# caomw/BundleAdjustmentMatlab

Measured on AMD Instinct MI355X. Metric: LM iterations/sec + observations/sec, 1000-cam/500k-pt synthetic, higher is better.
Workload: dtype f64; 1 GPU; cfg3: 1000 cams x 500000 pts x 3000000 obs, fix_calibration (num_a=6), full LM pass per step, one linearisation per step; cameras=1000, points=500000, observations=3000000, parallelism=point-shard x1

## Files before the change

bundleadjustmentmatlab_amd/bundle.py:

```python
from __future__ import annotations

import ctypes
import numpy as np

from ._lib import (ALLREDUCE_FN, LOSSES, MODEL_EUCLIDEAN, MODEL_PROJECTIVE, NKERNELS, ON_PASS_FN,
                   VlgbaOptions,
                   VlgbaProblem, VlgbaResectProblem, VlgbaStats,
                   VlgbaStepInfo, c_dp, c_ip, c_up, check, lib)

__all__ = ["bundle_euclid", "bundle_euclid_nomex", "bundle_euclid_obs", "BundleAdjuster",
           "bundle_euclid_resect",
           "parse_options", "pivot_mask",
           "mex_bundle_1_XABeUVWeAeB", "mex_bundle_2_Se_", "mex_bundle_3_db_new"]


def _F(a):
    return np.asfortranarray(a, dtype=np.float64)


def _dp(a):
    return a.ctypes.data_as(c_dp)


def pivot_mask(pivot, m):
# ... 320 lines not shown
        check(self._L.vlgba_set_timing(self._h, int(on)), "vlgba_set_timing")

    def kernel_ms(self, reset=True):
        n = NKERNELS
        ms = np.zeros(n)
        calls = (ctypes.c_longlong * n)()
        check(self._L.vlgba_kernel_ms(self._h, _dp(ms), calls, int(reset)), "vlgba_kernel_ms")
        return {self._L.vlgba_kernel_name(k).decode(): (float(ms[k]), int(calls[k]))
                for k in range(n) if calls[k] > 0}

    PLAN_KEYS = ("obs", "points", "cameras", "num_a", "chunks", "chunk_slots",
                 "chunk_eslots", "groups", "group_slots", "group_eslots", "blocks",
                 "tiles", "cr_levels", "cr_elim", "cr_keep", "ordered", "schur_terms",
                 "blob_words", "mfma", "cr_rows", "mfma_groups", "reordered", "long_points",
                 "nd_arcs", "nd_sep_tiles", "solve_flops_factor", "solve_flops_syrk",
                 "solve_flops_back", "env_runner_runs")

    def plan_info(self):
        n = len(self.PLAN_KEYS)
        buf = (ctypes.c_longlong * n)()
        rc = self._L.vlgba_plan_info(self._h, buf, n)
        check(min(rc, 0), "vlgba_plan_info")
        return dict(zip(self.PLAN_KEYS, [int(v) for v in buf]))

    def phase_ms(self):
        ms = np.zeros(7)
        check(self._L.vlgba_phase_ms(self._h, _dp(ms)), "vlgba_phase_ms")
        return dict(zip(["linearize", "camera_reduce", "damp_y", "schur", "assemble",
                         "cholesky_solve", "update"], ms.tolist()))


# ... 181 lines not shown
```

bundleadjustmentmatlab_amd/csrc/ba_chol.hip:

```cpp
#include "ba_internal.h"

#include <algorithm>
#include <atomic>
#include <mutex>
#include <cstdio>
#include <utility>
#include <climits>
#include <cstdlib>
#include <vector>

#define NB 64
#define LP 66

typedef double d4 __attribute__((ext_vector_type(4)));

__device__ __forceinline__ void load_tile(const double *__restrict__ S, long long lds, int ti,
                                          int tj, double *T)
{
    const double *base = S + (long long)NB * ti + lds * (long long)NB * tj;
    const int r = threadIdx.x & 63, c0 = threadIdx.x >> 6;
    double v[16];
#pragma unroll
    for (int u = 0; u < 16; u++) v[u] = base[r + lds * (c0 + 4 * u)];
#pragma unroll
// ... 2149 lines not shown
        }
    }
    __syncthreads();
}

__device__ __forceinline__ void cr32_publish(unsigned *flag, unsigned epoch, int nflags = 1)
{
    asm volatile("s_waitcnt vmcnt(0)" ::: "memory");
    __syncthreads();
    if (threadIdx.x < nflags)
        __hip_atomic_store((gu32_t *)(flag + threadIdx.x), epoch, __ATOMIC_RELAXED,
                           __HIP_MEMORY_SCOPE_AGENT);
}


__global__ __launch_bounds__(256) void k_cr32_fused(double *S, long long lds, int TB, long long ld,
                                                    const int *__restrict__ elim,
                                                    const int *__restrict__ frec,
                                                    const int *__restrict__ srec, int nt,
                                                    double *linv, double *crL, double *rhs,
                                                    double *y, double *x, unsigned *flag,
                                                    unsigned long long *xg, unsigned epoch,
                                                    double *status, cr32_fplan P)
{
    CR32_LDS_DECL;
    CR_ST(0);
    const int b = blockIdx.x;
    int L = 0;
    while (L < P.nl && b >= P.b0[L + 1]) L++;
    auto fw = [&](int lev, int t, int r) { return 5 * (lev * nt + t) + r; };
    if (L == 0) {
        const int xr = P.l0two ? b / 2 : b / 3;
        const int role = P.l0two ? ((b & 1) ? 2 : 4) : b % 3;
        const int e = elim[3 * xr], p = elim[3 * xr + 1], q = elim[3 * xr + 2];
        CR_ST(1);
        if (!((role == 1 && p < 0) || (role == 2 && q < 0)))
            cr32_factor_body<true>(sh, S, lds, TB, ld, e, p, q, role, nt, linv, crL, rhs, y,
                                   status);
// ... 59 lines not shown
        if (!skip)
            cr32_level_body<true>(sh, S, lds, TB, ld, k, p, q, em, ep, role, nt, linv, crL, rhs,
                                  y, status, mid, BA_CR_PW ? &pw : nullptr);
        CR_ST(2);
        cr32_publish(flag + fw(L, k, role == 3 ? 4 : role), epoch);
        CR_ST(3);
        return;
    }
    const int rec = P.nrec - 1 - (b - P.b0[P.nl]);
    int Le = 0;
    while (Le + 1 < P.nl && rec >= P.eofs[Le + 1]) Le++;
    const int e = elim[3 * rec], p = elim[3 * rec + 1], q = elim[3 * rec + 2];
    const int w[8] = {fw(Le, e, 0), fw(Le, e, 1), fw(Le, e, 2), 0, 0, 0, 0, 0};
    cr32_wait_flags(flag, 3, w, epoch, status);
    CR_ST(1);
    cr32_back_body<true>(sh, e, p, q, nt, TB, ld, linv, crL, y, x, xg, epoch, status);
    CR_ST(2);
    CR_ST(3);
}

__global__ __launch_bounds__(256) void k_cr_back(const int *__restrict__ elim, int nt,
                                                 const double *__restrict__ linv,
                                                 const double *__restrict__ crL,
                                                 const double *__restrict__ y,
                                                 double *__restrict__ x)
{
    __shared__ double Ls[NB * LP];
    __shared__ double t[NB], u[NB];
    __shared__ double part[4][NB];
    const int tid = threadIdx.x;
    const int e = elim[3 * blockIdx.x], p = elim[3 * blockIdx.x + 1], q = elim[3 * blockIdx.x + 2];
    const long long T2 = (long long)NB * NB;
// ... 912 lines not shown
        KT_E(d, KT_BACKWARD);
        return -(int)hipGetLastError();
    }
    for (int k = nt - 1; k >= 0; k--) {
        const int j0 = d->h_tfirst[k];
        KT_B(d);
        k_backward<<<k - j0 + 1, 256, 0, d->stream>>>(d->S, L, k, j0, d->linv, d->ywork, x);
        KT_E(d, KT_BACKWARD);
    }
    return -(int)hipGetLastError();
}

int ba_chol_solve(ba_dev *d, int nospin)
{
    const int nt = d->nt;
    const size_t smem3 = sizeof(double) * 3 * NB * LP;
    TRY_RC(ba_ensure_dyn_lds((const void *)k_factor_step, smem3));
    TRY_RC(ba_ensure_dyn_lds((const void *)k_cr_factor, smem3));
    TRY_RC(ba_ensure_dyn_lds((const void *)k_cr_update, smem3));
    if (d->dense_solve == 3) {
        KT_B(d);
        k_chol_seq<<<1, 256, 0, d->stream>>>(d->S, d->lds, (int)d->ld, d->rhs, d->da,
                                             d->scal + 4);
        KT_E(d, KT_FACTOR);
        return -(int)hipGetLastError();
    }
    if (d->cr_nlev > 0 && d->cr32 && d->cr_fused && d->crflag && !nospin) {
        const int nl = d->cr_nlev, nrec = d->cr_eptr_h[nl];
        cr32_fplan P{};
        P.nl = nl;
        P.nrec = nrec;
        P.l0two = 3 * d->cr_eptr_h[1] > d->ncu;
        P.b0[0] = 0;
        P.b0[1] = (P.l0two ? 2 : 3) * d->cr_eptr_h[1];
        for (int l = 1; l < nl; l++) {
            const int nf = d->crf_ptr_h[l + 1] - d->crf_ptr_h[l];
            const int ns = d->crs_ptr_h[l + 1] - d->crs_ptr_h[l];
            P.fofs[l] = d->crf_ptr_h[l];
            P.sofs[l] = d->crs_ptr_h[l];
            P.b0[l + 1] = P.b0[l] + 3 * nf + ns;
        }
        P.sofs[nl] = d->crs_ptr_h[nl];
        for (int l = 0; l <= nl; l++) P.eofs[l] = d->cr_eptr_h[l];
        if (++d->back_epoch == 0) d->back_epoch = 1;
        KT_B(d);
        k_cr32_fused<<<P.b0[nl] + nrec, 256, 0, d->stream>>>(
            d->S, d->lds, d->tb32, d->ld, d->cr_elim, d->crf, d->crs, d->nt32, d->linv, d->crL,
            d->rhs, d->ywork, d->da, d->crflag, d->xgran, d->back_epoch, d->scal + 4, P);
        KT_E(d, KT_CR_FACTOR);
        return -(int)hipGetLastError();
    }
    if (d->cr_nlev > 0 && d->cr32) {
        const int ncu32 = d->ncu;
        const int n32 = d->nt32, TB = d->tb32;
        {
            const int ne = d->cr_eptr_h[1];
            const int fs = 3 * ne <= 2 * ncu32;
            KT_B(d);
            k_cr32_factor<<<fs ? 3 * ne : ne, 256, 0, d->stream>>>(
                d->S, d->lds, TB, d->ld, d->cr_elim, n32, d->linv, d->crL, d->rhs, d->ywork,
                d->scal + 4, fs);
            KT_E(d, KT_CR_FACTOR);
        }
// ... 148 lines not shown
```

bundleadjustmentmatlab_amd/csrc/ba_internal.h:

```cpp
#pragma once
#include <hip/hip_runtime.h>
#include <cstddef>
#include <cstdint>

#define VLGBA_CHECK(x)                                                              \
    do {                                                                            \
        hipError_t err__ = (x);                                                     \
        if (err__ != hipSuccess) return -(int)err__;                                \
    } while (0)

enum {
    KT_ROT, KT_LIN, KT_CAMRED, KT_DAMP, KT_SCHUR, KT_SCHUR_CHUNK, KT_SCHUR_RED,
    KT_ASSEMBLE, KT_FACTOR, KT_SYRK, KT_BACKWARD, KT_CAMUPD, KT_PTUPD, KT_CR_FACTOR,
    KT_CR_UPDATE, KT_CR_BACK, KT_SCHUR_MF, KT_LIN_UPD, KT_N
};
#define KT_MAX_EV 8192
struct ba_ktimer {
    int on;
    int nev;
    int ncreated;
    hipEvent_t ev[KT_MAX_EV];
    int kid[KT_MAX_EV / 2];
    double ms[KT_N];
    long long calls[KT_N];
// ... 71 lines not shown
    int *tb_ptr, *tb_blk;
    int n_env;
    int dense_solve;
    int cr_nlev;
    int *cr_eptr_h, *cr_kptr_h;
    int *cr_elim, *cr_keep;
    double *crL;
    int cr32, tb32, nt32;
    int *crf, *crs;
    int *crf_ptr_h, *crs_ptr_h;
    unsigned long long *xgran;
    unsigned back_epoch;
    unsigned *crflag;
    int cr_fused;
    int asm_direct_ok, asm_direct;
    int nd_np;
    int nd_grouped;
    int nd_a0[BA_ND_MAX + 1];
    long long slds;
    int *nd_crow;
    int *nd_prow;
    int *nd_rowsrc;
    double *nd_rhs, *nd_x;
    int nd_npair, nd_nrec;
    int *nd_pair;
    int *nd_pptr;
    int *nd_rec;
    int *nd_klist;
    double *nd_part;
    double fl_factor, fl_syrk, fl_back;
// ... 22 lines not shown
    double *chsse;
    int fused;
    double *W2, *V2, *eB2, *upart2, *chsse2;
    int ns, nes;
    int ch_max_terms, ch_max_slots;
    long long nterm_fast;
    long long blob_words;
    int ngrp, ngs, nge;
    int grp_max_s, grp_max_e;
    unsigned *blob;
    int *ch_blob, *ch_obase;
    int *ch_cam;
    unsigned char *obs_lpt;
    int max_blob;
    int ngrp_mf;
    int nch_reg, nl, p_long;
    int *seg_pt, *seg_long;
    int *long_pt, *long_o0, *long_seg0;
    int *long_ebase;
    int *cam_lptr, *cam_lobs, *cam_ltrk;
    int max_lcam;
    int long_o0_h;
    double *ylong;
    int *lpair_ptr;
    int2 *lpair;
    int *lblk;
    int nlb;
    double *vseg;
    double *dpg_long;
    int mf_max_s, mf_max_e, mf_max_blob;
// ... 100 lines not shown
```

bundleadjustmentmatlab_amd/csrc/ba_kernels.hip:

```cpp
#include "ba_internal.h"
#include "ba_camera.h"
#include "vlg_math.h"
#include "../../include/vlgba.h"

typedef double d4 __attribute__((ext_vector_type(4)));

#ifdef BA_STAMPS
__device__ unsigned long long g_stamp[32];
#define STAMP_DECL unsigned long long st_prev_ = __builtin_amdgcn_s_memtime()
#define STAMP(i)                                                                    \
    do {                                                                            \
        if (threadIdx.x == 0) {                                                     \
            const unsigned long long t_ = __builtin_amdgcn_s_memtime();             \
            atomicAdd(&g_stamp[i], t_ - st_prev_);                                  \
            st_prev_ = t_;                                                          \
        }                                                                           \
    } while (0)
extern "C" int vlgba_debug_stamps(unsigned long long *out, int reset)
{
    if (hipMemcpyFromSymbol(out, HIP_SYMBOL(g_stamp), sizeof(g_stamp)) != hipSuccess) return -1;
    if (reset) {
        unsigned long long z[32] = {};
        if (hipMemcpyToSymbol(HIP_SYMBOL(g_stamp), z, sizeof(z)) != hipSuccess) return -1;
    }
// ... 1087 lines not shown
template <int Q> __device__ __forceinline__ double row16_bcast_c(double v)
{
    const long long u = __builtin_bit_cast(long long, v);
    const long long r = __builtin_amdgcn_mov_dpp(u, 0x150 + Q, 0xf, 0xf, true);
    return __builtin_bit_cast(double, r);
}
#ifndef BA_MF_WAVES
#define BA_MF_WAVES 3
#endif
template <int NA>
__global__ __launch_bounds__(256, (NA == 6) ? BA_MF_WAVES : 1) void k_schur_mfma(
    const int *__restrict__ grp_ch, const int *__restrict__ grp_gs,
    const int *__restrict__ grp_ge, const int *__restrict__ ch_pt,
    const int *__restrict__ ch_obase, const int *__restrict__ ch_blob,
    const unsigned *__restrict__ blob, const double *__restrict__ W,
    const double *__restrict__ Vinv, const double *__restrict__ eB, int nobs_all, int n_all,
    int gcap, int ecap, double *__restrict__ spart, double *__restrict__ epart, int ngrp,
    ba_camred cred)
{
    if ((int)blockIdx.x >= ngrp) {
        camera_reduce_wg<NA>((int)blockIdx.x - ngrp, cred);
        return;
    }
    constexpr int WS = 3 * NA;
    constexpr int RT = BA_MF_RT(NA);
    constexpr int NTL = RT * (RT + 1) / 2;
    extern __shared__ __attribute__((aligned(16))) double sm[];
    double *gacc = sm;
    double *geacc = gacc + gcap * NA * NA;
    unsigned *rec = (unsigned *)(geacc + ecap * NA);
    __shared__ int gp0[BA_GROUP_CH + 1], gob[BA_GROUP_CH + 1], gbo[BA_GROUP_CH + 1];
    const int g = ngrp - 1 - (int)blockIdx.x;
    const int tid = threadIdx.x, lane = tid & 63, wv = tid >> 6;
    const int li = lane & 15, lk = lane >> 4;
    const int c0 = grp_ch[g], nc = grp_ch[g + 1] - c0;
    const int gs0 = grp_gs[g], ngs = grp_gs[g + 1] - gs0;
    const int ge0 = grp_ge[g], nge = grp_ge[g + 1] - ge0;
    const int rb0 = ch_blob[c0], nrw = ch_blob[c0 + nc] - rb0;
    for (int q = tid; q < ngs * NA * NA; q += 256) gacc[q] = 0.0;
    for (int q = tid; q < nge * NA; q += 256) geacc[q] = 0.0;
    for (int q = tid; q < nrw; q += 256) rec[q] = blob[rb0 + q];
    for (int q = tid; q <= nc; q += 256) {
        gp0[q] = ch_pt[c0 + q];
        gob[q] = ch_obase[c0 + q];
        gbo[q] = ch_blob[c0 + q] - rb0;
    }
    __syncthreads();
    int ccs[RT], crr[RT];
#pragma unroll
    for (int t = 0; t < RT; t++) {
        ccs[t] = (16 * t + li) / NA;
        crr[t] = (16 * t + li) % NA;
    }
// ... 870 lines not shown
            b_new[3 * (size_t)i + r] = b[3 * (size_t)i + r] + dbr;
            dpg += dbr * (lambda * dbr + eB[3 * (size_t)i + r]);
        }
        dpg_long[l] = dpg;
    }
}

struct ba_sum3 {
    const double *part[3];
    int n[3];
    double *out[3];
    const double *scal;
    double *hres;
    double seq;
    unsigned *cnt;
};

__global__ __launch_bounds__(1024) void k_sum_parts3(ba_sum3 a)
{
    const double *part = a.part[blockIdx.x];
    const int nparts = a.n[blockIdx.x];
    double v0 = 0.0, v1 = 0.0, v2 = 0.0, v3 = 0.0;
    int q = threadIdx.x;
    for (; q + 3 * 1024 < nparts; q += 4 * 1024) {
        v0 += part[q];
        v1 += part[q + 1024];
        v2 += part[q + 2 * 1024];
        v3 += part[q + 3 * 1024];
    }
    for (; q < nparts; q += 1024) v0 += part[q];
    block_sum_to<1024>((v0 + v1) + (v2 + v3), a.out[blockIdx.x]);
    if (a.hres && threadIdx.x == 0) {
        __threadfence();
        if (atomicAdd(a.cnt, 1u) == 2u) {
            __threadfence();
            const volatile double *sc = a.scal;
// ... 145 lines not shown
                           d->blk_jk, d->blk_ptr, d->term, d->Y, d->W, d->t, d->U, d->eA, d->nb,
                           lambda, d->schur_owner, d->sblk, d->rhs)));
    KT_E(d, KT_SCHUR);
    return -(int)hipGetLastError();
}

#ifndef BA_SCHUR_TWO_STREAMS
#define BA_SCHUR_TWO_STREAMS 1
#endif
template <int NA>
static int launch_schur_fast(ba_dev *d, double lambda)
{
    const bool two = BA_SCHUR_TWO_STREAMS && d->ngrp_mf > 0 && d->ngrp > d->ngrp_mf &&
                     !d->join_pending && d->side && !(d->kt && d->kt->on);
    if (d->ngrp_mf > 0) {
        KT_B(d);
        k_point_vinv<NA><<<(d->n + 255) / 256, 256, 0, d->stream>>>(d->V, d->n, lambda, d->Vinv);
        KT_E(d, KT_DAMP);
        if (two) VLGBA_CHECK(hipEventRecord(d->ev_fork, d->stream));
        const size_t sm2 = sizeof(double) * (d->mf_max_s * NA * NA + d->mf_max_e * NA) +
                           sizeof(unsigned) * (size_t)d->mf_max_blob;
        TRY_RC(ba_ensure_dyn_lds((const void *)k_schur_mfma<NA>, sm2));
        const int ncr = d->camred_pending ? d->m + 1 : 0;
        d->camred_pending = 0;
        KT_B(d);
        k_schur_mfma<NA><<<d->ngrp_mf + ncr, 256, sm2, d->stream>>>(
            d->grp_ch, d->grp_gs, d->grp_ge, d->ch_pt, d->ch_obase, d->ch_blob, d->blob, d->W,
            d->Vinv, d->eB, d->N, d->n, d->mf_max_s, d->mf_max_e, d->spart, d->epart,
            d->ngrp_mf, d->camred);
        KT_E(d, KT_SCHUR_MF);
    }
    if (d->ngrp > d->ngrp_mf) {
        const int gcap = d->grp_max_s, ecap = d->grp_max_e, bcap = d->max_blob;
        size_t smem = sizeof(double) * (2 * BA_CH_OBS * 3 * NA + BA_CH_PTS * 12 +
                                        gcap * NA * NA + ecap * NA) +
                      sizeof(unsigned) * bcap;
        smem = (smem + 15) & ~(size_t)15;
        TRY_RC(ba_ensure_dyn_lds((const void *)k_schur_group<NA>, smem));
        hipStream_t s0 = d->stream;
        if (two) {
            VLGBA_CHECK(hipStreamWaitEvent(d->side, d->ev_fork, 0));
            d->stream = d->side;
        }
        KT_B(d);
// ... 86 lines not shown
    const int g = grid_for(d->n, 256, 1 << 30);
    BA_DISPATCH(d->na, (k_point_yeb<NA><<<g, 256, 0, d->stream>>>(d->pt_ptr, d->Y, d->eB, d->n,
                                                                    d->t)));
    return -(int)hipGetLastError();
}

int ba_launch_assemble(ba_dev *d)
{
    if (d->asm_direct) return 0;
    KT_B(d);
    TRY_RC(ba_assemble_tiles(d));
    KT_E(d, KT_ASSEMBLE);
    return 0;
}

static int launch_update_fused(ba_dev *d, double lambda, ba_flags f)
{
    const int gc = (d->m + 63) / 64;
    KT_B(d);
    const double lam_dpg = d->dpg_lambda ? lambda : 0.0;
    BA_DISPATCH(d->na, (k_camera_update<NA><<<gc, 320, 0, d->stream>>>(
                           d->a, d->da, d->eA, d->m, lam_dpg, d->a_new, d->rot_new,
                           d->part)));
    KT_E(d, KT_CAMUPD);
    KT_B(d);
    if (d->nl > 0)
        BA_DISPATCH(d->na, (k_long_db<NA><<<d->nl, 256, 0, d->stream>>>(
                               d->long_pt, d->long_o0, d->obs_cam, d->W, d->da, d->eB,
                               d->Vinv, d->b, d->ndb, lambda, d->db, d->b_new,
                               d->dpg_long)));
    const ba_upd u{d->W, d->da, d->eB, d->Vinv, d->b, d->ndb, lambda, d->db, d->b_new,
                   d->chsse2 + 2 * (size_t)d->nch, d->seg_long, d->long_o0, d->dpg_long};
    BA_DISPATCH(d->na, (lin_chunk_launch<NA>(d, f, d->a_new, d->rot_new, d->b_new, d->W2,
                                             d->V2, d->eB2, d->upart2, d->chsse2, &u)));
    if (d->nl > 0)
        k_long_vsum<<<d->nl, 64, 0, d->stream>>>(d->long_pt, d->long_seg0, d->vseg, d->V2,
                                                 d->eB2);
    KT_E(d, KT_LIN_UPD);
    ba_sum3 s3 = {{d->chsse2, d->chsse2 + 2 * (size_t)d->nch, d->part},
                  {d->nch, d->nch, gc},
                  {d->scal + 1, d->scal + 3, d->scal + 2},
                  d->scal, nullptr, 0.0, d->pub_cnt};
    if (d->publish_req) {
        d->seq++;
        s3.hres = d->hres_dev;
        s3.seq = (double)d->seq;
        d->publish_req = 0;
        d->published = 1;
    }
    k_sum_parts3<<<3, 1024, 0, d->stream>>>(s3);
    return -(int)hipGetLastError();
}

int ba_launch_update(ba_dev *d, double lambda, ba_flags f)
{
    if (d->fused) return launch_update_fused(d, lambda, f);
    const int gc = (d->m + 63) / 64;
    KT_B(d);
    const double lam_dpg = d->dpg_lambda ? lambda : 0.0;
    BA_DISPATCH(d->na, (k_camera_update<NA><<<gc, 320, 0, d->stream>>>(
                           d->a, d->da, d->eA, d->m, lam_dpg, d->a_new, d->rot_new,
                           d->part)));
    KT_E(d, KT_CAMUPD);
    if (!d->ordered && d->nch > 0 && !d->obs_vis && !d->xh_out) {
        KT_B(d);
        if (d->nl > 0)
            BA_DISPATCH(d->na, (k_long_db<NA><<<d->nl, 256, 0, d->stream>>>(
                                   d->long_pt, d->long_o0, d->obs_cam, d->W, d->da, d->eB,
                                   d->Vinv, d->b, d->ndb, lambda, d->db, d->b_new,
                                   d->dpg_long)));
        if (d->loss_kind) {
            const ba_loss ls{d->loss_kind, d->loss_scale};
            BA_DISPATCH(d->na, (k_point_update_chunk_loss<NA><<<d->nch, 256, 0, d->stream>>>(
                                   d->ch_pt, d->ch_obase, d->pt_ptr, d->obs_cam, d->obs_lpt,
                                   d->obs_x, d->K4, d->W, d->da, d->eB, d->Vinv, d->b,
                                   d->a_new, d->rot_new, d->ndb, lambda, d->db, d->b_new,
                                   d->chsse + d->nch, d->chsse + 2 * (size_t)d->nch,
                                   d->nch_reg, d->seg_pt, d->seg_long, d->long_o0,
                                   d->dpg_long, ls)));
        } else {
            BA_DISPATCH(d->na, (k_point_update_chunk<NA><<<d->nch, 256, 0, d->stream>>>(
                                   d->ch_pt, d->ch_obase, d->pt_ptr, d->obs_cam, d->obs_lpt,
                                   d->obs_x, d->K4, d->W, d->da, d->eB, d->Vinv, d->b,
                                   d->a_new, d->rot_new, d->ndb, lambda, d->db, d->b_new,
                                   d->chsse + d->nch, d->chsse + 2 * (size_t)d->nch,
                                   d->nch_reg, d->seg_pt, d->seg_long, d->long_o0,
                                   d->dpg_long)));
        }
        KT_E(d, KT_PTUPD);
        ba_sum3 s3 = {{d->chsse + d->nch, d->chsse + 2 * (size_t)d->nch, d->part},
                      {d->nch, d->nch, gc},
                      {d->scal + 1, d->scal + 3, d->scal + 2},
                      d->scal, nullptr, 0.0, d->pub_cnt};
        if (d->publish_req) {
            d->seq++;
            s3.hres = d->hres_dev;
            s3.seq = (double)d->seq;
            d->publish_req = 0;
            d->published = 1;
        }
        k_sum_parts3<<<3, 1024, 0, d->stream>>>(s3);
        return -(int)hipGetLastError();
    }
    k_sum_parts<<<1, BA_SUM_BS, 0, d->stream>>>(d->part, gc, d->scal + 2);
    const int g = grid_for(d->n, 256, PT_GRID_CAP);
    KT_B(d);
    BA_DISPATCH(d->na, (k_point_update<NA><<<g, 256, 0, d->stream>>>(
                           d->pt_ptr, d->obs_cam, d->obs_x, d->K4, d->W, d->da, d->eB, d->Vinv,
// ... 86 lines not shown
```

bundleadjustmentmatlab_amd/csrc/ba_solver.cpp:

```cpp
#include "ba_internal.h"
#include "../../include/vlgba.h"

#include <rccl/rccl.h>
#include <climits>
#include <rocsolver/rocsolver.h>

#include <dlfcn.h>
#include <unistd.h>
#include <cstdlib>
#include <string>

#include <algorithm>
#include <atomic>
#include <chrono>
#include <cmath>
#include <condition_variable>
#include <functional>
#include <cstdio>
#include <cstring>
#include <mutex>
#include <unordered_map>
#include <map>
#include <new>
#include <numeric>
// ... 1492 lines not shown
            TRY(ctx_alloc(c, &d.vseg, 12 * (size_t)plan.nseg));
            TRY(ctx_alloc(c, &d.dpg_long, (size_t)d.nl));
        }
        d.ns = (int)plan.slot_blk.size();
        d.nes = (int)plan.eslot_optr.size() - 1;
        d.ch_max_terms = plan.max_terms;
        d.ch_max_slots = plan.max_slots;
        d.nterm_fast = plan.n_terms;
        d.blob_words = (long long)plan.blob.size();
        d.ngrp = (int)plan.grp_ch.size() - 1;
        d.ngrp_mf = plan.ngrp_mf;
        d.max_blob = plan.max_blob;
        d.mf_max_blob = plan.mf_max_blob;
        d.mf_max_s = plan.mf_max_s;
        d.mf_max_e = plan.mf_max_e;
        pb.add(&d.blob, plan.blob);
        pb.add(&d.ch_blob, plan.ch_blob);
        pb.add(&d.ch_obase, plan.ch_obase);
        std::vector<unsigned char> lpt(d.N > 0 ? d.N : 1, 0);
        for (size_t ch = 0; ch + 1 < plan.ch_pt.size(); ch++)
            for (int i = plan.ch_pt[ch]; i < plan.ch_pt[ch + 1]; i++)
                for (int o = lptr[i]; o < lptr[i + 1]; o++)
                    lpt[o] = (unsigned char)(i - plan.ch_pt[ch]);
        const size_t nchk = plan.ch_obase.size() - 1;
        std::vector<int> ccam(2 * std::max<size_t>(nchk, 1), 0);
        for (size_t ch = 0; ch < nchk; ch++) {
            int lo = INT_MAX, hi = -1;
            for (int o = plan.ch_obase[ch]; o < plan.ch_obase[ch + 1]; o++) {
                lo = std::min(lo, lcam[o]);
                hi = std::max(hi, lcam[o]);
// ... 61 lines not shown
        TRY(ctx_alloc(c, &lp_cnt, (size_t)d.nb + 1));
        TRY(ctx_alloc(c, &d.lpair_ptr, (size_t)d.nb + 1));
        TRY(ba_launch_long_pairs(&d, 0, lp_cnt));
    }
    TRY(ctx_alloc(c, &d.sblk, (size_t)na * na * d.nb + d.lds + 1));
    d.rhs = d.sblk + (size_t)na * na * d.nb;
    if (!stage_mode) {
        TRY(ctx_alloc(c, &d.da, (size_t)d.lds));
        ST_MARK("allocs");
        TRY(ba_chol_setup(&d, hb.jk.data(), d.nb));
        ST_MARK("chol_setup");
        const char *ad = std::getenv("VLGBA_ASM_DIRECT");
        d.asm_direct = d.asm_direct_ok && !(ad && ad[0] == '0') && fast && !d.ordered &&
                       c->world == 1 && !c->comm && d.nl == 0 && d.cr_nlev > 0 && d.cr32 &&
                       d.nd_np == 0;
    } else {
        TRY(ctx_alloc(c, &d.da, (size_t)d.lds));
    }
    TRY(ctx_alloc(c, &d.part, 3 * (size_t)BA_PART_MAX));
    TRY(ctx_alloc(c, &d.scal, 8));
    if (p->num_obs > 0 || true) {
        TRY(upload(d.obs_cam, lcam.data(), d.N, s));
        TRY(upload(d.pt_ptr, lptr.data(), d.n + 1, s));
        TRY(upload(d.cam_ptr, cptr.data(), p->m + 1, s));
        TRY(upload(d.cam_obs, cobs.data(), d.N, s));
        TRY(upload(d.obs_x, h.x.data() + 2 * o0, 2 * (size_t)d.N, s));
        if (p->K) TRY(upload(d.K4, p->K, 4 * (size_t)p->m, s));
        else VLGBA_CHECK(hipMemsetAsync(d.K4, 0, sizeof(double) * 4 * p->m, s));
        TRY(upload(d.blk_ptr, hb.ptr.data(), hb.ptr.size(), s));
        TRY(upload(d.term, hb.term.data(), hb.term.size(), s));
// ... 346 lines not shown
    int info = 0;
    {
        std::lock_guard<std::mutex> lk(g_rs_mu);
        if (rs->set_stream(hdl, d.stream) != rocblas_status_success ||
            rs->potrf(hdl, rocblas_fill_lower, (rocblas_int)ld, c->pinv_S, (rocblas_int)ld,
                      c->pinv_info) != rocblas_status_success)
            return VLGBA_E_ARG;
        VLGBA_CHECK(hipMemcpyAsync(&info, c->pinv_info, sizeof info, hipMemcpyDeviceToHost,
                                   d.stream));
        VLGBA_CHECK(hipStreamSynchronize(d.stream));
        if (info != 0) return 1;
        if (rs->potrs(hdl, rocblas_fill_lower, (rocblas_int)ld, 1, c->pinv_S, (rocblas_int)ld,
                      c->pinv_e, (rocblas_int)ld) != rocblas_status_success)
            return VLGBA_E_ARG;
    }
    VLGBA_CHECK(hipMemcpyAsync(d.da, c->pinv_e, sizeof(double) * ld, hipMemcpyDeviceToDevice,
                               d.stream));
    d.publish_req = 0;
    d.published = 0;
    TRY(ba_launch_update(&d, lam, c->flags));
    if (d.parity) TRY(ba_launch_parity_new_sums(&d, lam));
    TRY(collect_scalars(c, false, hs));
    c->nd_retries++;
    if (c->rank == 0 && !std::getenv("VLGBA_QUIET"))
        std::fprintf(stderr, "[vlgba] non-positive pivot in the nested-dissection order: the "
                             "natural-order Cholesky (dpotrf) took the pass\n");
    return 0;
}

static int pinv_fallback(vlgba_ctx *c, double lam, double hs[6])
// ... 10 lines not shown
    {
        std::lock_guard<std::mutex> lk(g_rs_mu);
        if (rs->set_stream(hdl, d.stream) != rocblas_status_success ||
            rs->syevd(hdl, rocblas_evect_original, rocblas_fill_lower, (rocblas_int)ld,
                      c->pinv_S, (rocblas_int)ld, c->pinv_ev, c->pinv_e,
                      c->pinv_info) != rocblas_status_success)
            return VLGBA_E_ARG;
        VLGBA_CHECK(hipStreamSynchronize(d.stream));
    }
    {
        int info = 0;
        VLGBA_CHECK(hipMemcpy(&info, c->pinv_info, sizeof info, hipMemcpyDeviceToHost));
        if (info != 0) return VLGBA_E_ARG;
    }
    TRY(ba_pinv_apply(&d, c->pinv_S, c->pinv_ev, ld, d.rhs, c->pinv_w, d.da));
    d.publish_req = 0;
    d.published = 0;
    TRY(ba_launch_update(&d, lam, c->flags));
    if (d.parity) TRY(ba_launch_parity_new_sums(&d, lam));
    TRY(collect_scalars(c, false, hs));
    c->pinv_used++;
    if (c->rank == 0 && !std::getenv("VLGBA_QUIET"))
        std::fprintf(stderr,
                     "[vlgba] non-positive pivot: da = pinv(S) e_ by dsyevd on the dense "
                     "%lld x %lld S (%.1f MB of device memory), %.3f s\n",
                     ld, ld, 8e-6 * (double)ld * (double)ld,
                     std::chrono::duration<double>(std::chrono::steady_clock::now() - t0).count());
    return 0;
}

// ... 732 lines not shown

int vlgba_plan_info(vlgba_ctx *c, long long *info, int len)
{
    if (!c || !info) return VLGBA_E_ARG;
    const ba_dev &d = c->d;
    const long long ne = d.cr_nlev ? d.cr_eptr_h[d.cr_nlev] : 0;
    const long long nk = d.cr_nlev ? d.cr_kptr_h[d.cr_nlev] : 0;
    const long long v[VLGBA_NPLAN] = {d.N,   d.n,    d.m,   d.na,         d.nch,  d.ns,
                                      d.nes, d.ngrp, d.ngs, d.nge,        d.nb,   d.nt,
                                      d.cr_nlev, ne, nk,    d.ordered,    d.ordered ? d.T : d.nterm_fast,
                                      d.blob_words, d.mfma,
                                      d.cr_nlev ? (d.cr32 ? d.tb32 : 64) : 0,
                                      d.ngrp_mf, c->pperm.empty() ? 0 : 1, d.nl, d.nd_np,
                                      d.nd_np ? d.nt - d.nd_a0[d.nd_np] : 0,
                                      (long long)d.fl_factor, (long long)d.fl_syrk,
                                      (long long)d.fl_back, d.runner_runs};
    for (int k = 0; k < len && k < VLGBA_NPLAN; k++) info[k] = v[k];
    return VLGBA_NPLAN;
}

int vlgba_phase_ms(vlgba_ctx *c, double *ms7)
{
    if (!c || !ms7) return VLGBA_E_ARG;
    for (int q = 0; q < 7; q++) ms7[q] = c->phase_ms[q];
    return 0;
}

int vlgba_sync(vlgba_ctx *c)
{
    if (!c) return VLGBA_E_ARG;
    TRY(ctx_enter(c));
// ... 247 lines not shown
        const size_t p = (size_t)pt[q] + (size_t)n * cam[q];
        ox[2 * q] = X[2 * p];
        ox[2 * q + 1] = X[2 * p + 1];
        std::memcpy(hW.data() + bs * q, W + bs * p, sizeof(double) * bs);
    }
    vlgba_problem pr = {m, n, num_a, N, pt.data(), cam.data(), ox.data(), K, 0.0, model};
    vlgba_ctx *c = nullptr;
    TRY(ctx_create(&pr, nullptr, &c, true, true, true));
    ba_dev &d = c->d;
    int rc = 0;
    do {
        if ((rc = ctx_alloc(c, &d.xh_out, 2 * (size_t)N))) break;
        if ((rc = ctx_alloc(c, &d.obs_vis, (size_t)N))) break;
        if ((rc = upload(d.obs_vis, ov.data(), ov.size(), d.stream))) break;
        if ((rc = upload(d.W, hW.data(), hW.size(), d.stream))) break;
        if ((rc = upload(d.da, da, (size_t)d.ld, d.stream))) break;
        if ((rc = upload(d.eB, eB, 3 * (size_t)n, d.stream))) break;
        if ((rc = upload(d.Vinv, Vinv, 9 * (size_t)n, d.stream))) break;
        if ((rc = upload(d.a, a, (size_t)d.ld, d.stream))) break;
        if ((rc = upload(d.b, b, 3 * (size_t)n, d.stream))) break;
        VLGBA_CHECK(hipMemsetAsync(d.eA, 0, sizeof(double) * d.ld, d.stream));
        if ((rc = ba_launch_update(&d, 0.0, ba_flags{}))) break;
        if ((rc = download(db, d.db, 3 * (size_t)n, d.stream))) break;
        if ((rc = download(a_new, d.a_new, (size_t)d.ld, d.stream))) break;
        if ((rc = download(b_new, d.b_new, 3 * (size_t)n, d.stream))) break;
        if ((rc = download(xh.data(), d.xh_out, xh.size(), d.stream))) break;
        if (hipStreamSynchronize(d.stream) != hipSuccess) { rc = -1; break; }
    } while (0);
    ctx_free(c);
    if (rc) return rc;
// ... 112 lines not shown
```

include/vlgba.h:

```cpp
#ifndef VLGBA_H
#define VLGBA_H

#ifdef __cplusplus
extern "C" {
#endif

#define VLGBA_E_ARG (-1001)
#define VLGBA_E_NUMA (-1002)
#define VLGBA_E_ORDER (-1003)
#define VLGBA_E_NOMEM (-1004)
#define VLGBA_E_COMM (-1005)
#define VLGBA_E_ABI (-1006)
#define VLGBA_E_SINGULAR (-1007)

#define VLGBA_ABI_VERSION 6

#define VLGBA_MODEL_EUCLIDEAN 0
#define VLGBA_MODEL_PROJECTIVE 1

typedef struct {
    int m;
    int n;
    int num_a;
    long long num_obs;
// ... 73 lines not shown
                     double *cov_b, double *info);
#define VLGBA_LOSS_NONE 0
#define VLGBA_LOSS_HUBER 1
#define VLGBA_LOSS_CAUCHY 2
int vlgba_set_loss(vlgba_ctx *ctx, int kind, double scale);
int vlgba_get_loss(vlgba_ctx *ctx, int *kind, double *scale);
int vlgba_get_residuals(vlgba_ctx *ctx, double *e, double *w, double *rho);
int vlgba_sync(vlgba_ctx *ctx);
void vlgba_destroy(vlgba_ctx *ctx);
int vlgba_set_timing(vlgba_ctx *ctx, int on);
int vlgba_phase_ms(vlgba_ctx *ctx, double *ms7);
#define VLGBA_NKERNELS 18
int vlgba_kernel_ms(vlgba_ctx *ctx, double *ms, long long *calls, int reset);
int vlgba_kernel_flops(vlgba_ctx *ctx, double *flops);
const char *vlgba_kernel_name(int k);
#define VLGBA_NPLAN 29
int vlgba_plan_info(vlgba_ctx *ctx, long long *info, int len);


int vlgba_mex_bundle_1(int m, int n, int num_a, const double *K, const double *a,
                       const double *b, const double *X, const double *vis,
                       double *X_hat, double *A, double *B, double *e, double *U, double *V,
                       double *W, double *eA, double *eB);

int vlgba_mex_bundle_2(int m, int n, int num_a, const double *Y, const double *W,
                       const double *U, const double *eA, const double *eB, double *S,
                       double *e_);

int vlgba_mex_bundle_3(int m, int n, int num_a, const double *W, const double *da,
                       const double *eB, const double *Vinv, const double *K, const double *a,
                       const double *b, const double *X, const double *vis, double *db,
// ... 69 lines not shown
```

Measured before the change: 1949 LM iterations/s.

## Fold point Vinv damping into Schur kernel and camera update into CR back-solve

Measured after the change: 1974 LM iterations/s (median of 6 runs). 1.01x the previous value.

```diff
diff --git a/bundleadjustmentmatlab_amd/bundle.py b/bundleadjustmentmatlab_amd/bundle.py
--- a/bundleadjustmentmatlab_amd/bundle.py
+++ b/bundleadjustmentmatlab_amd/bundle.py
@@ -358,7 +358,7 @@
                  "tiles", "cr_levels", "cr_elim", "cr_keep", "ordered", "schur_terms",
                  "blob_words", "mfma", "cr_rows", "mfma_groups", "reordered", "long_points",
                  "nd_arcs", "nd_sep_tiles", "solve_flops_factor", "solve_flops_syrk",
-                 "solve_flops_back", "env_runner_runs")
+                 "solve_flops_back", "env_runner_runs", "vinv_fold", "camupd_fold")
 
     def plan_info(self):
         n = len(self.PLAN_KEYS)
diff --git a/bundleadjustmentmatlab_amd/csrc/ba_chol.hip b/bundleadjustmentmatlab_amd/csrc/ba_chol.hip
--- a/bundleadjustmentmatlab_amd/csrc/ba_chol.hip
+++ b/bundleadjustmentmatlab_amd/csrc/ba_chol.hip
@@ -1,4 +1,5 @@
 #include "ba_internal.h"
+#include "ba_camera.h"
 
 #include <algorithm>
 #include <atomic>
@@ -2187,6 +2188,12 @@
 }
 
 
+struct cr32_camupd {
+    const double *a;
+    double *a_new, *rot_new;
+    int na, m;
+};
+
 __global__ __launch_bounds__(256) void k_cr32_fused(double *S, long long lds, int TB, long long ld,
                                                     const int *__restrict__ elim,
                                                     const int *__restrict__ frec,
@@ -2194,7 +2201,8 @@
                                                     double *linv, double *crL, double *rhs,
                                                     double *y, double *x, unsigned *flag,
                                                     unsigned long long *xg, unsigned epoch,
-                                                    double *status, cr32_fplan P)
+                                                    double *status, cr32_fplan P,
+                                                    cr32_camupd cu)
 {
     CR32_LDS_DECL;
     CR_ST(0);
@@ -2284,8 +2292,27 @@
     const int w[8] = {fw(Le, e, 0), fw(Le, e, 1), fw(Le, e, 2), 0, 0, 0, 0, 0};
     cr32_wait_flags(flag, 3, w, epoch, status);
     CR_ST(1);
+    const int cl = threadIdx.x & 63, cc0 = cl / 5, ck = cl - 5 * cc0;
+    const int cj = (cu.a ? TB / cu.na : 0) * e + cc0;
+    const bool con = cu.a && (threadIdx.x >> 6) == 1 && cc0 < TB / cu.na && cj < cu.m;
+    double av[10];
+    if (con) {
+#pragma unroll
+        for (int cc = 0; cc < 10; cc++)
+            av[cc] = cc < cu.na ? cu.a[(size_t)cu.na * cj + cc] : 0.0;
+    }
     cr32_back_body<true>(sh, e, p, q, nt, TB, ld, linv, crL, y, x, xg, epoch, status);
     CR_ST(2);
+    if (con) {
+#pragma unroll
+        for (int cc = 0; cc < 10; cc++) {
+            if (cc < cu.na) {
+                av[cc] = av[cc] + sh.um[cu.na * cc0 + cc];
+                if (ck == 0) cu.a_new[(size_t)cu.na * cj + cc] = av[cc];
+            }
+        }
+        rotation_k(av, ck, cu.rot_new + 45 * (size_t)cj);
+    }
     CR_ST(3);
 }
 
@@ -3228,6 +3255,7 @@
 int ba_chol_solve(ba_dev *d, int nospin)
 {
     const int nt = d->nt;
+    d->camupd_done = 0;
     const size_t smem3 = sizeof(double) * 3 * NB * LP;
     TRY_RC(ba_ensure_dyn_lds((const void *)k_factor_step, smem3));
     TRY_RC(ba_ensure_dyn_lds((const void *)k_cr_factor, smem3));
@@ -3257,10 +3285,15 @@
         P.sofs[nl] = d->crs_ptr_h[nl];
         for (int l = 0; l <= nl; l++) P.eofs[l] = d->cr_eptr_h[l];
         if (++d->back_epoch == 0) d->back_epoch = 1;
+        cr32_camupd cu{};
+        if (d->camupd_fold) {
+            cu = cr32_camupd{d->a, d->a_new, d->rot_new, d->na, d->m};
+            d->camupd_done = 1;
+        }
         KT_B(d);
         k_cr32_fused<<<P.b0[nl] + nrec, 256, 0, d->stream>>>(
             d->S, d->lds, d->tb32, d->ld, d->cr_elim, d->crf, d->crs, d->nt32, d->linv, d->crL,
-            d->rhs, d->ywork, d->da, d->crflag, d->xgran, d->back_epoch, d->scal + 4, P);
+            d->rhs, d->ywork, d->da, d->crflag, d->xgran, d->back_epoch, d->scal + 4, P, cu);
         KT_E(d, KT_CR_FACTOR);
         return -(int)hipGetLastError();
     }
diff --git a/bundleadjustmentmatlab_amd/csrc/ba_internal.h b/bundleadjustmentmatlab_amd/csrc/ba_internal.h
--- a/bundleadjustmentmatlab_amd/csrc/ba_internal.h
+++ b/bundleadjustmentmatlab_amd/csrc/ba_internal.h
@@ -109,6 +109,7 @@
     unsigned *crflag;
     int cr_fused;
     int asm_direct_ok, asm_direct;
+    int camupd_fold, camupd_done;
     int nd_np;
     int nd_grouped;
     int nd_a0[BA_ND_MAX + 1];
@@ -161,6 +162,7 @@
     unsigned char *obs_lpt;
     int max_blob;
     int ngrp_mf;
+    int vinv_fold;
     int nch_reg, nl, p_long;
     int *seg_pt, *seg_long;
     int *long_pt, *long_o0, *long_seg0;
diff --git a/bundleadjustmentmatlab_amd/csrc/ba_kernels.hip b/bundleadjustmentmatlab_amd/csrc/ba_kernels.hip
--- a/bundleadjustmentmatlab_amd/csrc/ba_kernels.hip
+++ b/bundleadjustmentmatlab_amd/csrc/ba_kernels.hip
@@ -1125,9 +1125,9 @@
     const int *__restrict__ grp_ge, const int *__restrict__ ch_pt,
     const int *__restrict__ ch_obase, const int *__restrict__ ch_blob,
     const unsigned *__restrict__ blob, const double *__restrict__ W,
-    const double *__restrict__ Vinv, const double *__restrict__ eB, int nobs_all, int n_all,
+    double *Vinv, const double *__restrict__ eB, int nobs_all, int n_all,
     int gcap, int ecap, double *__restrict__ spart, double *__restrict__ epart, int ngrp,
-    ba_camred cred)
+    ba_camred cred, const double *__restrict__ Vdamp, double lambda)
 {
     if ((int)blockIdx.x >= ngrp) {
         camera_reduce_wg<NA>((int)blockIdx.x - ngrp, cred);
@@ -1148,6 +1148,40 @@
     const int gs0 = grp_gs[g], ngs = grp_gs[g + 1] - gs0;
     const int ge0 = grp_ge[g], nge = grp_ge[g + 1] - ge0;
     const int rb0 = ch_blob[c0], nrw = ch_blob[c0 + nc] - rb0;
+    if (Vdamp) {
+        const int p0 = ch_pt[c0], p1 = ch_pt[c0 + nc];
+        double t[9];
+        auto rows = [&](int i0) {
+            const int cnt = 9 * min(256, p1 - i0);
+            const double *src = Vdamp + 9 * (size_t)i0;
+#pragma unroll
+            for (int u = 0; u < 9; u++) t[u] = tid + 256 * u < cnt ? src[tid + 256 * u] : 0.0;
+        };
+        if (p0 < p1) rows(p0);
+        for (int i0 = p0; i0 < p1; i0 += 256) {
+            const int cnt = 9 * min(256, p1 - i0);
+#pragma unroll
+            for (int u = 0; u < 9; u++) sm[tid + 256 * u] = t[u];
+            __syncthreads();
+            if (i0 + 256 < p1) rows(i0 + 256);
+            if (i0 + tid < p1) {
+                double vs[9], vi[9];
+#pragma unroll
+                for (int q = 0; q < 9; q++) vs[q] = sm[9 * tid + q];
+#pragma unroll
+                for (int c = 0; c < 3; c++) vs[4 * c] = (1 + lambda) * vs[4 * c];
+                vlg_pinv3(vs, vi);
+#pragma unroll
+                for (int q = 0; q < 9; q++) sm[9 * tid + q] = vi[q];
+            }
+            __syncthreads();
+            double *dst = Vinv + 9 * (size_t)i0;
+#pragma unroll
+            for (int u = 0; u < 9; u++)
+                if (tid + 256 * u < cnt) dst[tid + 256 * u] = sm[tid + 256 * u];
+            __syncthreads();
+        }
+    }
     for (int q = tid; q < ngs * NA * NA; q += 256) gacc[q] = 0.0;
     for (int q = tid; q < nge * NA; q += 256) geacc[q] = 0.0;
     for (int q = tid; q < nrw; q += 256) rec[q] = blob[rb0 + q];
@@ -2048,12 +2082,33 @@
     double *hres;
     double seq;
     unsigned *cnt;
+    const double *cam_da, *cam_eA;
+    double *cam_part;
+    int cam_m, cam_na;
+    double cam_lambda;
 };
 
 __global__ __launch_bounds__(1024) void k_sum_parts3(ba_sum3 a)
 {
     const double *part = a.part[blockIdx.x];
     const int nparts = a.n[blockIdx.x];
+    if (blockIdx.x == 2 && a.cam_da) {
+        const int lane = threadIdx.x & 63;
+        for (int g = threadIdx.x >> 6; g < nparts; g += 16) {
+            const int j = 64 * g + lane;
+            double acc = 0.0;
+            if (j < a.cam_m) {
+                for (int c = 0; c < a.cam_na; c++) {
+                    const double d = a.cam_da[(size_t)a.cam_na * j + c];
+                    acc += d * (a.cam_lambda * d + a.cam_eA[(size_t)a.cam_na * j + c]);
+                }
+            }
+#pragma unroll
+            for (int off = 32; off > 0; off >>= 1) acc += __shfl_down(acc, off, 64);
+            if (lane == 0) a.cam_part[g] = acc;
+        }
+        __syncthreads();
+    }
     double v0 = 0.0, v1 = 0.0, v2 = 0.0, v3 = 0.0;
     int q = threadIdx.x;
     for (; q + 3 * 1024 < nparts; q += 4 * 1024) {
@@ -2229,12 +2284,17 @@
     const bool two = BA_SCHUR_TWO_STREAMS && d->ngrp_mf > 0 && d->ngrp > d->ngrp_mf &&
                      !d->join_pending && d->side && !(d->kt && d->kt->on);
     if (d->ngrp_mf > 0) {
-        KT_B(d);
-        k_point_vinv<NA><<<(d->n + 255) / 256, 256, 0, d->stream>>>(d->V, d->n, lambda, d->Vinv);
-        KT_E(d, KT_DAMP);
+        if (!d->vinv_fold) {
+            KT_B(d);
+            k_point_vinv<NA><<<(d->n + 255) / 256, 256, 0, d->stream>>>(d->V, d->n, lambda,
+                                                                        d->Vinv);
+            KT_E(d, KT_DAMP);
+        }
         if (two) VLGBA_CHECK(hipEventRecord(d->ev_fork, d->stream));
-        const size_t sm2 = sizeof(double) * (d->mf_max_s * NA * NA + d->mf_max_e * NA) +
-                           sizeof(unsigned) * (size_t)d->mf_max_blob;
+        size_t sm2 = sizeof(double) * (d->mf_max_s * NA * NA + d->mf_max_e * NA) +
+                     sizeof(unsigned) * (size_t)d->mf_max_blob;
+        if (d->vinv_fold && sm2 < sizeof(double) * 256 * 9)
+            sm2 = sizeof(double) * 256 * 9;
         TRY_RC(ba_ensure_dyn_lds((const void *)k_schur_mfma<NA>, sm2));
         const int ncr = d->camred_pending ? d->m + 1 : 0;
         d->camred_pending = 0;
@@ -2242,7 +2302,7 @@
         k_schur_mfma<NA><<<d->ngrp_mf + ncr, 256, sm2, d->stream>>>(
             d->grp_ch, d->grp_gs, d->grp_ge, d->ch_pt, d->ch_obase, d->ch_blob, d->blob, d->W,
             d->Vinv, d->eB, d->N, d->n, d->mf_max_s, d->mf_max_e, d->spart, d->epart,
-            d->ngrp_mf, d->camred);
+            d->ngrp_mf, d->camred, d->vinv_fold ? d->V : nullptr, lambda);
         KT_E(d, KT_SCHUR_MF);
     }
     if (d->ngrp > d->ngrp_mf) {
@@ -2359,15 +2419,27 @@
     return 0;
 }
 
-static int launch_update_fused(ba_dev *d, double lambda, ba_flags f)
+static void sum3_camera_dpg(ba_dev *d, double lam_dpg, ba_sum3 *s3)
+{
+    s3->cam_da = d->da;
+    s3->cam_eA = d->eA;
+    s3->cam_part = d->part;
+    s3->cam_m = d->m;
+    s3->cam_na = d->na;
+    s3->cam_lambda = lam_dpg;
+}
+
+static int launch_update_fused(ba_dev *d, double lambda, ba_flags f, bool folded)
 {
     const int gc = (d->m + 63) / 64;
-    KT_B(d);
     const double lam_dpg = d->dpg_lambda ? lambda : 0.0;
-    BA_DISPATCH(d->na, (k_camera_update<NA><<<gc, 320, 0, d->stream>>>(
-                           d->a, d->da, d->eA, d->m, lam_dpg, d->a_new, d->rot_new,
-                           d->part)));
-    KT_E(d, KT_CAMUPD);
+    if (!folded) {
+        KT_B(d);
+        BA_DISPATCH(d->na, (k_camera_update<NA><<<gc, 320, 0, d->stream>>>(
+                               d->a, d->da, d->eA, d->m, lam_dpg, d->a_new, d->rot_new,
+                               d->part)));
+        KT_E(d, KT_CAMUPD);
+    }
     KT_B(d);
     if (d->nl > 0)
         BA_DISPATCH(d->na, (k_long_db<NA><<<d->nl, 256, 0, d->stream>>>(
@@ -2386,6 +2458,7 @@
                   {d->nch, d->nch, gc},
                   {d->scal + 1, d->scal + 3, d->scal + 2},
                   d->scal, nullptr, 0.0, d->pub_cnt};
+    if (folded) sum3_camera_dpg(d, lam_dpg, &s3);
     if (d->publish_req) {
         d->seq++;
         s3.hres = d->hres_dev;
@@ -2399,15 +2472,20 @@
 
 int ba_launch_update(ba_dev *d, double lambda, ba_flags f)
 {
-    if (d->fused) return launch_update_fused(d, lambda, f);
+    const bool chunked = !d->ordered && d->nch > 0 && !d->obs_vis && !d->xh_out;
+    const bool folded = d->camupd_done && (d->fused || chunked);
+    d->camupd_done = 0;
+    if (d->fused) return launch_update_fused(d, lambda, f, folded);
     const int gc = (d->m + 63) / 64;
-    KT_B(d);
     const double lam_dpg = d->dpg_lambda ? lambda : 0.0;
-    BA_DISPATCH(d->na, (k_camera_update<NA><<<gc, 320, 0, d->stream>>>(
-                           d->a, d->da, d->eA, d->m, lam_dpg, d->a_new, d->rot_new,
-                           d->part)));
-    KT_E(d, KT_CAMUPD);
-    if (!d->ordered && d->nch > 0 && !d->obs_vis && !d->xh_out) {
+    if (!folded) {
+        KT_B(d);
+        BA_DISPATCH(d->na, (k_camera_update<NA><<<gc, 320, 0, d->stream>>>(
+                               d->a, d->da, d->eA, d->m, lam_dpg, d->a_new, d->rot_new,
+                               d->part)));
+        KT_E(d, KT_CAMUPD);
+    }
+    if (chunked) {
         KT_B(d);
         if (d->nl > 0)
             BA_DISPATCH(d->na, (k_long_db<NA><<<d->nl, 256, 0, d->stream>>>(
@@ -2437,6 +2515,7 @@
                       {d->nch, d->nch, gc},
                       {d->scal + 1, d->scal + 3, d->scal + 2},
                       d->scal, nullptr, 0.0, d->pub_cnt};
+        if (folded) sum3_camera_dpg(d, lam_dpg, &s3);
         if (d->publish_req) {
             d->seq++;
             s3.hres = d->hres_dev;
diff --git a/bundleadjustmentmatlab_amd/csrc/ba_solver.cpp b/bundleadjustmentmatlab_amd/csrc/ba_solver.cpp
--- a/bundleadjustmentmatlab_amd/csrc/ba_solver.cpp
+++ b/bundleadjustmentmatlab_amd/csrc/ba_solver.cpp
@@ -1530,6 +1530,17 @@
         d.mf_max_blob = plan.mf_max_blob;
         d.mf_max_s = plan.mf_max_s;
         d.mf_max_e = plan.mf_max_e;
+        {
+            bool tile = d.ngrp_mf > 0 && d.ngrp == d.ngrp_mf && d.nl == 0;
+            int at = 0;
+            for (int g = 0; tile && g < d.ngrp_mf; g++) {
+                tile = plan.ch_pt[plan.grp_ch[g]] == at &&
+                       plan.ch_pt[plan.grp_ch[g + 1]] >= at;
+                at = plan.ch_pt[plan.grp_ch[g + 1]];
+            }
+            const char *vf = std::getenv("VLGBA_VINV_FOLD");
+            d.vinv_fold = tile && at == d.n && !(vf && vf[0] == '0');
+        }
         pb.add(&d.blob, plan.blob);
         pb.add(&d.ch_blob, plan.ch_blob);
         pb.add(&d.ch_obase, plan.ch_obase);
@@ -1621,6 +1632,11 @@
         d.asm_direct = d.asm_direct_ok && !(ad && ad[0] == '0') && fast && !d.ordered &&
                        c->world == 1 && !c->comm && d.nl == 0 && d.cr_nlev > 0 && d.cr32 &&
                        d.nd_np == 0;
+        const char *cf = std::getenv("VLGBA_CAMUPD_FOLD");
+        d.camupd_fold = !(cf && cf[0] == '0') && fast && !d.ordered && d.nch > 0 &&
+                        d.cr_nlev > 0 && d.cr32 && d.cr_fused && d.crflag && d.nd_np == 0 &&
+                        na != BA_PROJ_NA && na <= 10 && d.tb32 % na == 0 &&
+                        d.ld == (long long)na * p->m;
     } else {
         TRY(ctx_alloc(c, &d.da, (size_t)d.lds));
     }
@@ -1997,6 +2013,7 @@
                       c->pinv_e, (rocblas_int)ld) != rocblas_status_success)
             return VLGBA_E_ARG;
     }
+    d.camupd_done = 0;
     VLGBA_CHECK(hipMemcpyAsync(d.da, c->pinv_e, sizeof(double) * ld, hipMemcpyDeviceToDevice,
                                d.stream));
     d.publish_req = 0;
@@ -2037,6 +2054,7 @@
         if (info != 0) return VLGBA_E_ARG;
     }
     TRY(ba_pinv_apply(&d, c->pinv_S, c->pinv_ev, ld, d.rhs, c->pinv_w, d.da));
+    d.camupd_done = 0;
     d.publish_req = 0;
     d.published = 0;
     TRY(ba_launch_update(&d, lam, c->flags));
@@ -2799,7 +2817,8 @@
                                       d.ngrp_mf, c->pperm.empty() ? 0 : 1, d.nl, d.nd_np,
                                       d.nd_np ? d.nt - d.nd_a0[d.nd_np] : 0,
                                       (long long)d.fl_factor, (long long)d.fl_syrk,
-                                      (long long)d.fl_back, d.runner_runs};
+                                      (long long)d.fl_back, d.runner_runs, d.vinv_fold,
+                                      d.camupd_fold};
     for (int k = 0; k < len && k < VLGBA_NPLAN; k++) info[k] = v[k];
     return VLGBA_NPLAN;
 }
@@ -3077,6 +3096,7 @@
         if ((rc = ctx_alloc(c, &d.obs_vis, (size_t)N))) break;
         if ((rc = upload(d.obs_vis, ov.data(), ov.size(), d.stream))) break;
         if ((rc = upload(d.W, hW.data(), hW.size(), d.stream))) break;
+        d.camupd_done = 0;
         if ((rc = upload(d.da, da, (size_t)d.ld, d.stream))) break;
         if ((rc = upload(d.eB, eB, 3 * (size_t)n, d.stream))) break;
         if ((rc = upload(d.Vinv, Vinv, 9 * (size_t)n, d.stream))) break;
diff --git a/include/vlgba.h b/include/vlgba.h
--- a/include/vlgba.h
+++ b/include/vlgba.h
@@ -111,7 +111,7 @@
 int vlgba_kernel_ms(vlgba_ctx *ctx, double *ms, long long *calls, int reset);
 int vlgba_kernel_flops(vlgba_ctx *ctx, double *flops);
 const char *vlgba_kernel_name(int k);
-#define VLGBA_NPLAN 29
+#define VLGBA_NPLAN 31
 int vlgba_plan_info(vlgba_ctx *ctx, long long *info, int len);
 
 
```
